# virtualsecureplatform/cuFHE

Hardware: AMD Instinct MI355X
Metric: nand_gate_bootstraps_per_sec (higher is better)
Workload: dtype f64

## Files before the change

### cufhe_amd/csrc/fpfield.h

```cpp
#pragma once
#include <stdint.h>

#if (defined(CUFHE_AMD_ABL_NO_TW) || defined(CUFHE_AMD_ABL_NO_XPOSE) || defined(CUFHE_AMD_ABL_NO_BK) || \
     defined(CUFHE_AMD_ABL_BK0) || defined(CUFHE_AMD_ABL_NO_SYNC) || defined(CUFHE_AMD_ABL_PHASES) || defined(CUFHE_AMD_ABL_LL2_TIMEOUT) || defined(CUFHE_AMD_ABL_L2_NOATOM)) && !defined(CUFHE_AMD_DIAGNOSTIC_BUILD)
#error "CUFHE_AMD_ABL_* switches produce wrong results: use `python cufhe_amd/build.py --diagnostic=NAME[,NAME]` (defines CUFHE_AMD_DIAGNOSTIC_BUILD, output libcufhe_amd_diag.so)"
#endif

#if defined(__HIPCC__)
#define FPF_HD __host__ __device__ __forceinline__
#else
#define FPF_HD static inline
#endif

namespace fpf {

constexpr uint64_t ZETA8 = 5440ull;
constexpr uint64_t P_U64 = 875781160960001ull;
constexpr uint64_t PSI_2048 = 423584205157050ull;
constexpr double P = 875781160960001.0;
constexpr double PINV = 0x1.491cc17c934a8p-50;
constexpr double ROOT4 = 29593600.0;
constexpr double ROOT8 = 5440.0;
constexpr double INV_ROOT4 = 0x1.22436485a6c7fp-25;
constexpr double MAGIC0 = 6755399441055744.0;
constexpr double MAGIC1 = 13510798882111488.0;

FPF_HD double mulmod(double a, double w)
{
    const double h = a * w;
    const double l = __builtin_fma(a, w, -h);
    const double q = __builtin_fma(h, PINV, MAGIC0) - MAGIC0;
    const double r = __builtin_fma(-q, P, h);
    return r + l;
}
FPF_HD double mulmod_wide(double a, double w)
{
    const double h = a * w;
    const double l = __builtin_fma(a, w, -h);
    const double q = __builtin_fma(h, PINV, MAGIC1) - MAGIC1;
    const double r = __builtin_fma(-q, P, h);
    return r + l;
}
FPF_HD double mulmod_add(double a, double w, double c)
{
    const double h = a * w;
    const double l = __builtin_fma(a, w, -h);
    const double q = __builtin_fma(h + c, PINV, MAGIC0) - MAGIC0;
    const double r = __builtin_fma(-q, P, h);
    return (r + c) + l;
}
FPF_HD double mulmod_add_wide(double a, double w, double c)
{
    const double h = a * w;
    const double l = __builtin_fma(a, w, -h);
    const double q = __builtin_fma(h + c, PINV, MAGIC1) - MAGIC1;
    const double r = __builtin_fma(-q, P, h);
    return (r + c) + l;
}
FPF_HD double mul_root4(double x)
{
    const double x1 = __builtin_fma(x, INV_ROOT4, MAGIC0) - MAGIC0;
    const double x0 = __builtin_fma(-x1, ROOT4, x);
    return __builtin_fma(x0, ROOT4, -x1);
}
FPF_HD double reduce(double a)
{
    const double q = __builtin_fma(a, PINV, MAGIC0) - MAGIC0;
    return __builtin_fma(-q, P, a);
}
FPF_HD uint32_t low32(double a)
{
    const double t = a + MAGIC0;
    uint64_t bits;
    __builtin_memcpy(&bits, &t, 8);
    return (uint32_t)bits;
}
FPF_HD uint32_t lift_u32(double a) { return low32(reduce(a)); }
FPF_HD uint32_t lift_u32_small(double a)
{
    const double t = __builtin_fma(a, PINV, MAGIC0);
    uint64_t tb;
    __builtin_memcpy(&tb, &t, 8);
    return low32(a) - (uint32_t)tb * (uint32_t)P_U64;
}


constexpr double GROW = 0.09723;
constexpr double LIM_NARROW = 5.142;
constexpr double LIM_WIDE = 10.285;
constexpr double after_mulmod(double a) { return 0.5 + GROW * a; }
constexpr double after_mulmod_wide(double a) { return 1.0 + GROW * a; }
constexpr double GROW_ADD = 0.14585;
constexpr double after_mulmod_add(double a) { return 0.5 + GROW_ADD * a; }
constexpr double after_mulmod_add_wide(double a) { return 1.0 + GROW_ADD * a; }
constexpr double AFTER_MUL_ROOT4 = 0.5000005;

}
```

### cufhe_amd/csrc/kernels.hip.h

```cpp
#pragma once
#include "kernels_common.hip.h"

namespace cufhe_amd {

__global__ __launch_bounds__(kNttThreads) void bk_to_ntt_kernel(
    double* __restrict__ bk_ntt, const uint32_t* __restrict__ bk, size_t polys,
    const NttTables* __restrict__ gt, double n_inverse)
{
    extern __shared__ __attribute__((aligned(16))) char smem[];
    double* tabs = (double*)smem;
    load_tables_to_lds(tabs, gt);
    __syncthreads();
    const int wave = threadIdx.x >> 6, lane = threadIdx.x & 63;
    const size_t poly = (size_t)blockIdx.x * kNttWavesPerBlock + wave;
    if (poly >= polys) return;
    const WaveCtx ctx = make_wave_ctx(smem, kLdsTableBytes + wave * kTileBytes, 0, gt, lane);
    double x[kRegs];
#pragma unroll
    for (int r = 0; r < kRegs; r++) x[r] = (double)(int32_t)bk[poly * kN + lane + 64 * r];
    ntt_forward<false>(x, ctx);
    double2* dst = (double2*)(bk_ntt + poly * kN);
#pragma unroll
    for (int q = 0; q < 8; q++) {
        double2 v;
        v.x = fpf::reduce(fpf::mulmod_wide(x[2 * q], n_inverse));
        v.y = fpf::reduce(fpf::mulmod_wide(x[2 * q + 1], n_inverse));
        dst[q * 64 + lane] = v;
    }
}

__global__ __launch_bounds__(512) void clock_probe_kernel(double* __restrict__ hz_out, double* __restrict__ sink, int iters)
{
    double x = 1.0 + threadIdx.x * 1e-9, y = 0.5;
    const unsigned long long c0 = __builtin_amdgcn_s_memtime(), r0 = __builtin_amdgcn_s_memrealtime();
#pragma unroll 1
    for (int i = 0; i < iters; i++) {
#pragma unroll
        for (int k = 0; k < 16; k++) { x = __builtin_fma(x, 0.999999, y); y = __builtin_fma(y, 0.999999, x); }
    }
    const unsigned long long c1 = __builtin_amdgcn_s_memtime(), r1 = __builtin_amdgcn_s_memrealtime();
    if (x + y == 12345.678) sink[0] = x;
    if ((threadIdx.x & 63) == 0)
        hz_out[blockIdx.x * (blockDim.x >> 6) + (threadIdx.x >> 6)] = (double)(c1 - c0) / (double)(r1 - r0) * 1.0e8;
}

__device__ __forceinline__ void rotate_sub(uint32_t (&temp)[kRegs], const uint32_t (&acc)[kRegs],
                                           char* tile, int lane, uint32_t abar)
{
    const int alo = (int)(abar & (kN - 1));
    const bool ahi = (abar >> kNbit) != 0;
    char* wpos = tile + opaque(4 * lane + (ahi ? 0 : 4 * kN));
    char* wneg = tile + opaque(4 * lane + (ahi ? 4 * kN : 0));
    asm volatile("" ::: "memory");
#pragma unroll
    for (int r = 0; r < kRegs; r++) {
        *(uint32_t*)(wpos + 256 * r) = acc[r];
        *(uint32_t*)(wneg + 256 * r) = 0u - acc[r];
    }
    asm volatile("" ::: "memory");
    const char* rbase = tile + opaque(4 * (lane - alo + kN));
    uint32_t rot[kRegs];
#pragma unroll
    for (int r = 0; r < kRegs; r++) rot[r] = *(const uint32_t*)(rbase + 256 * r);
#pragma unroll
    for (int r = 0; r < kRegs; r++) temp[r] = (rot[r] - acc[r] + decomp_offset()) ^ decomp_signmask();
}

template <class SPEC, int R, bool LAST, bool FIRST = false>
__device__ __forceinline__ void product_into(double& acc, double x, double w)
{
    constexpr bool wide = r4::needs_wide(SPEC::in().v[R]);
    static_assert(!(LAST && FIRST), "a sum of one product has no first row apart from its last");
    if constexpr (LAST) acc = wide ? fpf::mulmod_add_wide(x, w, acc) : fpf::mulmod_add(x, w, acc);
    else if constexpr (FIRST) acc = wide ? fpf::mulmod_wide(x, w) : fpf::mulmod(x, w);
    else acc += wide ? fpf::mulmod_wide(x, w) : fpf::mulmod(x, w);
}
template <class SPEC, bool LAST, bool FIRST, int Q>
__device__ __forceinline__ void pointwise_piece(double (&A0)[kRegs], double (&A1)[kRegs], const double (&x)[kRegs], const double2& b)
{
    if constexpr (Q < 8) {
        product_into<SPEC, 2 * Q, LAST, FIRST>(A0[2 * Q], x[2 * Q], b.x);
        product_into<SPEC, 2 * Q + 1, LAST, FIRST>(A0[2 * Q + 1], x[2 * Q + 1], b.y);
    } else {
        product_into<SPEC, 2 * (Q - 8), LAST, FIRST>(A1[2 * (Q - 8)], x[2 * (Q - 8)], b.x);
        product_into<SPEC, 2 * (Q - 8) + 1, LAST, FIRST>(A1[2 * (Q - 8) + 1], x[2 * (Q - 8) + 1], b.y);
    }
}
template <class SPEC, bool LAST, bool FIRST, int Q = 0>
__device__ __forceinline__ void pointwise_pieces(double (&A0)[kRegs], double (&A1)[kRegs], const double (&x)[kRegs],
                                                 double2 (&b)[16], const char* row_lane)
{
#ifndef CUFHE_AMD_BK_DEPTH
#define CUFHE_AMD_BK_DEPTH 3
#endif
    constexpr int D = CUFHE_AMD_BK_DEPTH;
    if constexpr (Q < 16) {
        if constexpr (Q + D < 16) b[Q + D] = *(const double2*)(row_lane + (Q + D) * 1024);
        __builtin_amdgcn_sched_barrier(0x0006);
        pointwise_piece<SPEC, LAST, FIRST, Q>(A0, A1, x, b[Q]);
        __builtin_amdgcn_sched_barrier(0x0006);
        pointwise_pieces<SPEC, LAST, FIRST, Q + 1>(A0, A1, x, b, row_lane);
    }
}
template <class SPEC, bool LAST, bool FIRST = false>
__device__ __forceinline__ void pointwise_accumulate(double (&A0)[kRegs], double (&A1)[kRegs],
                                                     const double (&x)[kRegs], const char* row_lane)
{
#if defined(CUFHE_AMD_DIAGNOSTIC_BUILD) && defined(CUFHE_AMD_ABL_NO_BK)
    if constexpr (FIRST) {
#pragma unroll
        for (int r = 0; r < kRegs; r++) { A0[r] = 0.0; A1[r] = 0.0; }
    }
#pragma unroll
    for (int q = 0; q < 8; q++) {
        A0[2 * q] += fpf::mulmod_wide(x[2 * q], 1234567.0 + q);
        A0[2 * q + 1] += fpf::mulmod_wide(x[2 * q + 1], 7654321.0 + q);
        A1[2 * q] += fpf::mulmod_wide(x[2 * q], 2234567.0 + q);
        A1[2 * q + 1] += fpf::mulmod_wide(x[2 * q + 1], 8654321.0 + q);
    }
    (void)row_lane;
    return;
#endif
    constexpr int D = CUFHE_AMD_BK_DEPTH;
    double2 b[16];
#pragma unroll
    for (int q = 0; q < D; q++) b[q] = *(const double2*)(row_lane + q * 1024);
    pointwise_pieces<SPEC, LAST, FIRST>(A0, A1, x, b, row_lane);
}

#if defined(CUFHE_AMD_DIAGNOSTIC_BUILD) && defined(CUFHE_AMD_ABL_PHASES)
#define CUFHE_AMD_DIAG_ARG , unsigned long long& diag_wait
#define CUFHE_AMD_DIAG_PASS , diag_wait
#define CUFHE_AMD_ROW_SYNC(R) { const unsigned long long t0_ = __builtin_readcyclecounter(); pipe.sync(R); diag_wait += __builtin_readcyclecounter() - t0_; }
#else
#define CUFHE_AMD_DIAG_ARG
#define CUFHE_AMD_DIAG_PASS
#define CUFHE_AMD_ROW_SYNC(R) pipe.sync(R);
#endif
struct RowPipe {
    const char* src;
    char* buf;
    uint32_t voff;
    int wave, lane, total_rows;
    bool late;
    int row_off;
    __device__ __forceinline__ RowPipe(const char* bk, char* buf_, int wave_, int lane_, int total_rows_, bool late_)
        : src(bk + 2 * wave_ * 1024), buf(buf_), voff(lane_ * 16), wave(wave_), lane(lane_), total_rows(total_rows_), late(late_),
          row_off((kBkRowBuffers - 1) * kBkRowBytes) {}
    static __device__ __forceinline__ int next_off(int off) { return off == (kBkRowBuffers - 1) * kBkRowBytes ? 0 : off + kBkRowBytes; }
    __device__ __forceinline__ void issue(int R)
    {
        if (R < total_rows) {
            char* dst = buf + next_off(row_off) + 2 * wave * 1024;
#pragma unroll
            for (int c = 0; c < 2; c++) lds_dma16(src + c * 1024, voff, dst + c * 1024);
        }
        src += kBkRowBytes;
    }
    __device__ __forceinline__ void sync(int R)
    {
#if defined(CUFHE_AMD_DIAGNOSTIC_BUILD) && defined(CUFHE_AMD_ABL_NO_SYNC)
        (void)R;
        return;
#endif
        lds_dma_wait_all();
        __syncthreads();
        row_off = next_off(row_off);
        issue(R + 1);
    }
    __device__ __forceinline__ const char* row() const { return buf + opaque(row_off + lane * 16); }
};

using BrSpectrum = r4::FwdDigits<(1 << (kBgbit - 1))>::Spectrum;
using BrSums = r4::PointwiseSum<BrSpectrum, kBkRows, true>;
using BrInverse = r4::Inverse<BrSums>;
static_assert(r4::valid(BrSpectrum::in()) && r4::valid(BrSums::in()) && r4::valid(BrInverse::Out::in()),
              "blind_rotate_kernel: the lazy-reduction schedule of the CMux step exceeds the FP64 mantissa");

template <bool FIRST, bool LAST>
__device__ __forceinline__ void cmux_row(double (&A0)[kRegs], double (&A1)[kRegs], const uint32_t (&temp)[kRegs], int d,
                                         const WaveCtx& ctx, RowPipe& pipe, int row, const TuFwdPinned& tuf CUFHE_AMD_DIAG_ARG)
{
    constexpr int kDigitMax = 1 << (kBgbit - 1);
    const uint32_t pos = 32 - (d + 1) * kBgbit;
    double x[kRegs];
#pragma unroll
    for (int r = 0; r < kRegs; r++)
        x[r] = (double)(int32_t)__builtin_amdgcn_sbfe(temp[r], pos, (uint32_t)kBgbit);
    double twb[kTbCount];
    ntt_forward_digits_a_r4<kDigitMax, true>(x, ctx, &tuf, &twb);
    if (pipe.late) CUFHE_AMD_ROW_SYNC(row)
    ntt_forward_digits_bc_r4<kDigitMax, false, true>(x, ctx, twb);
    if (!pipe.late) CUFHE_AMD_ROW_SYNC(row)
    pointwise_accumulate<BrSpectrum, LAST, FIRST>(A0, A1, x, pipe.row());
}

template <bool FIRST_COMPONENT, bool LAST_COMPONENT>
__device__ __forceinline__ void cmux_component(double (&A0)[kRegs], double (&A1)[kRegs],
                                               const uint32_t (&accj)[kRegs], const WaveCtx& ctx,
                                               char* tile, int lane, uint32_t abar,
                                               RowPipe& pipe, int first_row, const TuFwdPinned& tuf CUFHE_AMD_DIAG_ARG)
{
    uint32_t temp[kRegs];
    rotate_sub(temp, accj, tile, lane, abar);
    static_assert(kL >= 2, "the first and the last row of a component are two rows");
    constexpr int lo = FIRST_COMPONENT ? 1 : 0, hi = LAST_COMPONENT ? kL - 1 : kL;
    if constexpr (FIRST_COMPONENT) cmux_row<true, false>(A0, A1, temp, 0, ctx, pipe, first_row, tuf CUFHE_AMD_DIAG_PASS);
#pragma unroll 1
    for (int d = lo; d < hi; d++) cmux_row<false, false>(A0, A1, temp, d, ctx, pipe, first_row + d, tuf CUFHE_AMD_DIAG_PASS);
    if constexpr (LAST_COMPONENT) cmux_row<false, true>(A0, A1, temp, kL - 1, ctx, pipe, first_row + kL - 1, tuf CUFHE_AMD_DIAG_PASS);
}

template <bool TWB_LOADED>
__device__ __forceinline__ void inverse_and_add(double (&A)[kRegs], uint32_t (&accj)[kRegs], const WaveCtx& ctx,
                                                const double (&twc)[kTcCount], double (&twb)[kTbCount])
{
    ntt_inverse_r4_tw<BrSums, false, TWB_LOADED>(A, ctx, twc, twb);
    lift_add<BrInverse::Out>(accj, A);
}

template <bool TABLE>
__global__ __launch_bounds__(kBrThreads, 2) void blind_rotate_kernel(
    const LinDesc* __restrict__ descs, int count, const double* __restrict__ bk_ntt,
    const NttTables* __restrict__ gt, int steps, uint32_t* __restrict__ acc_dump, int active, const uint32_t* __restrict__ tvs,
    const uint32_t* const* __restrict__ tables)
{
    extern __shared__ __attribute__((aligned(16))) char smem[];
    double* tabs = (double*)(smem + kBrLdsTables);
    load_packed_tables_to_lds(tabs, gt);
    const int wave = __builtin_amdgcn_readfirstlane(threadIdx.x >> 6);
    const int lane = threadIdx.x & 63;
    const int g = blockIdx.x * active + wave;
    char* tile = smem + kBrLdsTiles + wave * kTileBytes;
    uint16_t* abar_lds = (uint16_t*)(smem + kBrLdsAbar + wave * kAbarBytes);
    const WaveCtx ctx = make_wave_ctx_packed(smem, kBrLdsTiles + wave * kTileBytes, kBrLdsTables, gt, lane);
    RowPipe pipe((const char*)bk_ntt, smem + kBrLdsBk, wave, lane, steps * kBkRows, wave >= kBrWavesPerBlock / 2);
    pipe.issue(0);
    if (wave >= active || g >= count) {
        __syncthreads();
#pragma unroll 1
        for (int R = 0; R < pipe.total_rows; R++) pipe.sync(R);
        return;
    }

    const LinDesc d = descs[g];
    uint32_t bword = 0;
#pragma unroll
    for (int rr = 0; rr < 10; rr++) {
        const int i = lane + 64 * rr;
        uint32_t c = 0;
        if (i <= kLvl0N) c = (uint32_t)d.ca * d.in0[i] + (uint32_t)d.cb * d.in1[i];
        if (rr == 9) bword = c;
        if (i < kLvl0N) abar_lds[i] = (uint16_t)((c + (1u << (32 - 2 - kNbit))) >> (32 - 1 - kNbit));
    }
    bword = __builtin_amdgcn_readlane(bword, kLvl0N - 64 * 9) + d.off;
    const uint32_t bbar = 2 * kN - (bword >> (32 - 1 - kNbit));

    uint32_t acc0[kRegs], acc1[kRegs];
#pragma unroll
    for (int r = 0; r < kRegs; r++) {
        const uint32_t e = lane + 64 * r;
        acc0[r] = 0;
        const bool neg = (bbar != 2 * kN) && ((e < (bbar & (kN - 1))) != ((bbar >> kNbit) != 0));
        acc1[r] = neg ? 0u - kMu : kMu;
    }
    const uint32_t* tab = nullptr;
    if constexpr (TABLE) tab = tables[g];
    if (TABLE && tab) {
        const int s = desc_shift(d.pad);
        uint32_t bb = bbar;
        if (s) {
            for (int i = lane; i < kLvl0N; i += 64) abar_lds[i] = (uint16_t)ms_abar((uint32_t)d.ca * d.in0[i] + (uint32_t)d.cb * d.in1[i], s);
            bb = ms_bbar(bword, s);
        }
#pragma unroll
        for (int r = 0; r < kRegs; r++) {
            acc0[r] = rotated_tv_coef(tab, bb, lane + 64 * r);
            acc1[r] = rotated_tv_coef(tab + kN, bb, lane + 64 * r);
        }
    } else if (d.pad) {
        const uint32_t* tv = desc_tv(tvs, d.pad);
        const int s = desc_shift(d.pad);
        uint32_t bb = bbar;
        if (s) {
            for (int i = lane; i < kLvl0N; i += 64) abar_lds[i] = (uint16_t)ms_abar((uint32_t)d.ca * d.in0[i] + (uint32_t)d.cb * d.in1[i], s);
            bb = ms_bbar(bword, s);
        }
#pragma unroll
        for (int r = 0; r < kRegs; r++) acc1[r] = rotated_tv_coef(tv, bb, lane + 64 * r);
    }
    __syncthreads();
    TuFwdPinned tuf;
    tuf.load(gt);
#if defined(CUFHE_AMD_DIAGNOSTIC_BUILD) && defined(CUFHE_AMD_ABL_PHASES)
    unsigned long long diag_wait = 0;
    const unsigned long long diag_t0 = __builtin_readcyclecounter();
#endif

#pragma unroll 1
    for (int i = 0; i < steps; i++) {
        const uint32_t abar = __builtin_amdgcn_readfirstlane((uint32_t)abar_lds[i]);
        double A0[kRegs], A1[kRegs], inv_twc[kTcCount], inv_twb[kTbCount];
        cmux_component<true, false>(A0, A1, acc0, ctx, tile, lane, abar, pipe, i * kBkRows, tuf CUFHE_AMD_DIAG_PASS);
        cmux_component<false, true>(A0, A1, acc1, ctx, tile, lane, abar, pipe, i * kBkRows + kL, tuf CUFHE_AMD_DIAG_PASS);
        load_packed(inv_twc, ctx.tc_inv);
        inverse_and_add<false>(A0, acc0, ctx, inv_twc, inv_twb);
        inverse_and_add<true>(A1, acc1, ctx, inv_twc, inv_twb);
    }

    if (acc_dump) {
        uint32_t* o = acc_dump + (size_t)g * 2 * kN;
#pragma unroll
        for (int r = 0; r < kRegs; r++) {
            o[lane + 64 * r] = acc0[r];
            o[kN + lane + 64 * r] = acc1[r];
        }
#if defined(CUFHE_AMD_DIAGNOSTIC_BUILD) && defined(CUFHE_AMD_ABL_PHASES)
        if (lane == 0) {
            ((unsigned long long*)o)[0] = __builtin_readcyclecounter() - diag_t0;
            ((unsigned long long*)o)[1] = diag_wait;
        }
#endif
    }
    if (d.out) {
        uint32_t* o = d.out;
#pragma unroll
        for (int r = 0; r < kRegs; r++) {
            const int e = lane + 64 * r;
            if (e == 0) { o[0] = acc0[r]; o[kN] = acc1[r]; }
            else o[kN - e] = 0u - acc0[r];
        }
        if (const int s = desc_shift(d.pad)) {
#pragma unroll
            for (int r = 0; r < kRegs; r++) extract_more(o, 1 << s, lane + 64 * r, acc0[r], acc1[r]);
        }
    }
}

constexpr int kKsWaves = 16;
constexpr int kKsThreads = 64 * kKsWaves;
constexpr int kKsRowPad = 640;
constexpr int kKsPieces = 3;
constexpr int kKsStepBytes = kKsT * kKsNumBase * kKsRowPad * 4;
constexpr int kKsBuffers = 3;
constexpr int kKsDigitSteps = 1024;
constexpr int kKsLdsDigits = kKsWaves * kKsDigitSteps * 2;

struct KsShapeDefault {
    using Desc = LinDesc;
    static constexpr int kn = kN, t = kKsT, row_pad = kKsRowPad, n_out = kLvl0N;
    static constexpr uint32_t koff()
    {
        uint32_t o = 1u << (32 - (1 + kKsBasebit * kKsT));
        for (int i = 1; i <= kKsT; i++) o += ((1u << kKsBasebit) / 2) << (32 - i * kKsBasebit);
        return o;
    }
    static __device__ __forceinline__ uint32_t digit_word(const Desc& d, int j)
    {
        return ((uint32_t)d.ca * d.in0[j] + (uint32_t)d.cb * d.in1[j] + koff()) >> 16;
    }
    static __device__ __forceinline__ uint32_t bprime(const Desc& d) { return (uint32_t)d.ca * d.in0[kn] + (uint32_t)d.cb * d.in1[kn] + d.off; }
};
template <class S>
struct KsDims {
    static constexpr int pairs = (S::row_pad - 512) / 128;
    static constexpr int words = 8 + 2 * pairs;
    static constexpr int step_bytes = S::t * kKsNumBase * S::row_pad * 4;
    static constexpr int dma_pieces = step_bytes / 1024;
    static constexpr int dma_more = dma_pieces - 2 * kKsWaves;
    static constexpr int lds_bytes = kKsLdsDigits + kKsBuffers * step_bytes;
    static constexpr int min_slices = (S::kn + kKsDigitSteps - 1) / kKsDigitSteps;
// ... 503 lines not shown
```

### cufhe_amd/csrc/ntt_r4.h

```cpp
#pragma once
#include "fpfield.h"

#if defined(__HIPCC__)
#define R4_HD __host__ __device__ __forceinline__
#else
#define R4_HD inline
#endif

namespace cufhe_amd {
namespace r4 {

struct RegBounds {
    double v[16];
};
constexpr double kPoison = 1.0e30;
constexpr double kReduced = 0.5001;

constexpr RegBounds uniform(double b)
{
    RegBounds r{};
    for (int i = 0; i < 16; i++) r.v[i] = b;
    return r;
}
constexpr double max_of(const RegBounds& b)
{
    double m = 0;
    for (int i = 0; i < 16; i++) m = b.v[i] > m ? b.v[i] : m;
    return m;
}
constexpr bool valid(const RegBounds& b) { return max_of(b) < fpf::LIM_WIDE; }
constexpr bool needs_wide(double b) { return b >= fpf::LIM_NARROW; }
constexpr double after_product(double b)
{
    return b >= fpf::LIM_WIDE ? kPoison : needs_wide(b) ? fpf::after_mulmod_wide(b) : fpf::after_mulmod(b);
}
constexpr double checked(double b) { return b >= fpf::LIM_WIDE ? kPoison : b; }

template <bool HI>
constexpr int reg_of(int group, int coarse, int fine)
{
    return HI ? group + 8 * coarse + 4 * fine : 4 * group + 2 * coarse + fine;
}

template <bool HI>
constexpr RegBounds ct_bounds(const RegBounds& in)
{
    RegBounds out{};
    for (int g = 0; g < 4; g++) {
        const double a = in.v[reg_of<HI>(g, 0, 0)];
        const double mb = after_product(in.v[reg_of<HI>(g, 1, 0)]);
        const double mc = after_product(in.v[reg_of<HI>(g, 0, 1)]);
        const double md = after_product(in.v[reg_of<HI>(g, 1, 1)]);
        const double sum = checked(checked(a + mb) + checked(mc + md));
        const double dif = checked(checked(a + mb) + fpf::AFTER_MUL_ROOT4);
        out.v[reg_of<HI>(g, 0, 0)] = sum;
        out.v[reg_of<HI>(g, 0, 1)] = sum;
        out.v[reg_of<HI>(g, 1, 0)] = dif;
        out.v[reg_of<HI>(g, 1, 1)] = dif;
    }
    return out;
}
template <bool HI>
constexpr RegBounds gs_bounds(const RegBounds& in)
{
    RegBounds out{};
    for (int g = 0; g < 4; g++) {
        const double s0 = checked(in.v[reg_of<HI>(g, 0, 0)] + in.v[reg_of<HI>(g, 0, 1)]);
        const double s1 = checked(in.v[reg_of<HI>(g, 1, 0)] + in.v[reg_of<HI>(g, 1, 1)]);
        out.v[reg_of<HI>(g, 0, 0)] = checked(s0 + s1);
        out.v[reg_of<HI>(g, 1, 0)] = after_product(checked(s0 + s1));
        out.v[reg_of<HI>(g, 0, 1)] = after_product(checked(s0 + fpf::AFTER_MUL_ROOT4));
        out.v[reg_of<HI>(g, 1, 1)] = after_product(checked(s0 + fpf::AFTER_MUL_ROOT4));
    }
    return out;
}
constexpr RegBounds xpose_all_bounds(const RegBounds& in) { return uniform(max_of(in)); }
constexpr RegBounds xpose_bc_bounds(const RegBounds& in)
{
    RegBounds out{};
    for (int m = 0; m < 4; m++) {
        double mx = 0;
        for (int h = 0; h < 4; h++) mx = in.v[4 * h + m] > mx ? in.v[4 * h + m] : mx;
        for (int g = 0; g < 4; g++) out.v[4 * m + g] = mx;
    }
    return out;
}
constexpr RegBounds xpose_cb_bounds(const RegBounds& in)
{
    RegBounds out{};
    for (int m = 0; m < 4; m++) {
        double mx = 0;
        for (int g = 0; g < 4; g++) mx = in.v[4 * m + g] > mx ? in.v[4 * m + g] : mx;
        for (int h = 0; h < 4; h++) out.v[4 * h + m] = mx;
    }
    return out;
}
constexpr RegBounds reduce_bounds(const RegBounds& in, double limit)
{
    RegBounds out = in;
    for (int r = 0; r < 16; r++)
        if (in.v[r] > limit) out.v[r] = kReduced;
    return out;
}
constexpr RegBounds reduce_mask_bounds(const RegBounds& in, unsigned mask)
{
    RegBounds out = in;
    for (int r = 0; r < 16; r++)
        if ((mask >> r) & 1u) out.v[r] = kReduced;
    return out;
}

template <class S, bool HI>
struct AfterCt {
    static constexpr RegBounds in() { return ct_bounds<HI>(S::in()); }
};
template <class S, bool HI>
struct AfterGs {
    static constexpr RegBounds in() { return gs_bounds<HI>(S::in()); }
};
template <class S>
struct AfterXposeAll {
    static constexpr RegBounds in() { return xpose_all_bounds(S::in()); }
};
template <class S>
struct AfterXposeBC {
    static constexpr RegBounds in() { return xpose_bc_bounds(S::in()); }
};
template <class S>
struct AfterXposeCB {
    static constexpr RegBounds in() { return xpose_cb_bounds(S::in()); }
};
template <class S, int LIMIT_MILLI>
struct AfterReduce {
    static constexpr RegBounds in() { return reduce_bounds(S::in(), LIMIT_MILLI * 0.001); }
};
template <class S, unsigned MASK>
struct AfterReduceMask {
    static constexpr RegBounds in() { return reduce_mask_bounds(S::in(), MASK); }
};
template <int MILLI>
struct Uniform {
    static constexpr RegBounds in() { return uniform(MILLI * 0.001); }
};

template <int DIGIT_MAX>
struct DigitsAfterExact {
    static constexpr RegBounds in()
    {
        const double s1 = DIGIT_MAX * (1.0 + fpf::ROOT4 + fpf::ROOT8 + fpf::ROOT8 * fpf::ROOT8 * fpf::ROOT8);
        return uniform(s1 < 9007199254740992.0 / 64.0 ? s1 / fpf::P : kPoison);
    }
};
template <int DIGIT_MAX>
struct FwdDigits {
    using A0 = DigitsAfterExact<DIGIT_MAX>;
    using B0 = AfterXposeAll<AfterCt<A0, false>>;
    using B1 = AfterCt<B0, true>;
    using C0 = AfterXposeBC<AfterCt<B1, false>>;
    static constexpr unsigned kReduceC = 0x1111u;
    using C1 = AfterReduceMask<C0, kReduceC>;
    using Spectrum = AfterCt<C1, false>;
};
template <class SPEC, int ROWS, bool FUSED>
struct PointwiseSum {
    static constexpr RegBounds in()
    {
        RegBounds out{};
        const RegBounds s = SPEC::in();
        for (int r = 0; r < 16; r++) {
            const double prod = after_product(s.v[r]);
            if (FUSED) {
                const double last = s.v[r] >= fpf::LIM_WIDE ? kPoison : needs_wide(s.v[r]) ? fpf::after_mulmod_add_wide(s.v[r]) : fpf::after_mulmod_add(s.v[r]);
                out.v[r] = checked((ROWS - 1) * prod + last) >= kPoison ? kPoison : last;
            } else {
                out.v[r] = checked(ROWS * prod);
            }
        }
        return out;
    }
};

template <class S0>
struct Inverse {
    static constexpr int kLimit = 2570;
    using C1 = AfterGs<S0, false>;
    using B0 = AfterXposeCB<AfterReduce<C1, kLimit>>;
    using B1 = AfterReduce<AfterGs<B0, false>, kLimit>;
    using B2 = AfterReduce<AfterGs<B1, true>, kLimit>;
    using A0 = AfterXposeAll<B2>;
    using A1 = AfterReduce<AfterGs<A0, false>, kLimit>;
    using Out = AfterGs<A1, true>;
};

template <bool WIDE>
R4_HD double product(double a, double w) { return WIDE ? fpf::mulmod_wide(a, w) : fpf::mulmod(a, w); }

template <bool WB, bool WC, bool WD>
R4_HD void ct_bfly4(double& x0, double& xf, double& xc, double& xcf, double w, double u, double uw)
{
    const double b = product<WB>(xc, w), c = product<WC>(xf, u), d = product<WD>(xcf, uw);
    const double s = x0 + b, e = x0 - b, t = c + d, v = fpf::mul_root4(c - d);
    x0 = s + t;
    xf = s - t;
    xc = e + v;
    xcf = e - v;
}
template <bool WC, bool WF, bool WCF>
R4_HD void gs_bfly4(double& x0, double& xf, double& xc, double& xcf, double w, double v, double vw)
{
    const double s0 = x0 + xf, p = x0 - xf, s1 = xc + xcf, q = fpf::mul_root4(xc - xcf);
    x0 = s0 + s1;
    xc = product<WC>(s0 - s1, w);
    xf = product<WF>(p - q, v);
    xcf = product<WCF>(p + q, vw);
}

template <class S, bool HI, int G>
struct Group {
    static constexpr RegBounds b = S::in();
    static constexpr int r0 = reg_of<HI>(G, 0, 0), rf = reg_of<HI>(G, 0, 1), rc = reg_of<HI>(G, 1, 0), rcf = reg_of<HI>(G, 1, 1);
    static R4_HD void ct(double (&x)[16], double w, double u, double uw)
    {
        ct_bfly4<needs_wide(b.v[rc]), needs_wide(b.v[rf]), needs_wide(b.v[rcf])>(x[r0], x[rf], x[rc], x[rcf], w, u, uw);
    }
    static R4_HD void gs(double (&x)[16], double w, double v, double vw)
    {
        constexpr double s0 = b.v[r0] + b.v[rf], s1 = b.v[rc] + b.v[rcf];
        gs_bfly4<needs_wide(s0 + s1), needs_wide(s0 + fpf::AFTER_MUL_ROOT4), needs_wide(s0 + fpf::AFTER_MUL_ROOT4)>(x[r0], x[rf], x[rc], x[rcf], w, v, vw);
    }
};

template <class S, class TW>
R4_HD void ct_pass_hi(double (&x)[16], const TW& tw)
{
    const double w = tw(0), u = tw(1), uw = tw(2);
    Group<S, true, 0>::ct(x, w, u, uw);
    Group<S, true, 1>::ct(x, w, u, uw);
    Group<S, true, 2>::ct(x, w, u, uw);
    Group<S, true, 3>::ct(x, w, u, uw);
}
template <class S, int WB, int UB, class TW>
R4_HD void ct_pass_lo(double (&x)[16], const TW& tw)
{
    Group<S, false, 0>::ct(x, tw(WB + 0), tw(UB + 0), tw(UB + 1));
    Group<S, false, 1>::ct(x, tw(WB + 1), tw(UB + 2), tw(UB + 3));
    Group<S, false, 2>::ct(x, tw(WB + 2), tw(UB + 4), tw(UB + 5));
    Group<S, false, 3>::ct(x, tw(WB + 3), tw(UB + 6), tw(UB + 7));
}
template <class S, class TW>
R4_HD void gs_pass_hi(double (&x)[16], const TW& tw)
{
    const double w = tw(0), v = tw(1), vw = tw(2);
    Group<S, true, 0>::gs(x, w, v, vw);
    Group<S, true, 1>::gs(x, w, v, vw);
    Group<S, true, 2>::gs(x, w, v, vw);
    Group<S, true, 3>::gs(x, w, v, vw);
}
template <class S, int WB, int UB, class TW>
R4_HD void gs_pass_lo(double (&x)[16], const TW& tw)
{
    Group<S, false, 0>::gs(x, tw(WB + 0), tw(UB + 0), tw(UB + 1));
    Group<S, false, 1>::gs(x, tw(WB + 1), tw(UB + 2), tw(UB + 3));
    Group<S, false, 2>::gs(x, tw(WB + 2), tw(UB + 4), tw(UB + 5));
    Group<S, false, 3>::gs(x, tw(WB + 3), tw(UB + 6), tw(UB + 7));
}
template <class S, int LIMIT_MILLI, int R = 0>
R4_HD void reduce_above(double (&x)[16])
{
    if constexpr (R < 16) {
        if constexpr (S::in().v[R] > LIMIT_MILLI * 0.001) x[R] = fpf::reduce(x[R]);
        reduce_above<S, LIMIT_MILLI, R + 1>(x);
    }
}

template <class S, int LIMIT_MILLI, int G>
R4_HD void reduce_above_group(double (&x)[16])
{
    if constexpr (S::in().v[G] > LIMIT_MILLI * 0.001) x[G] = fpf::reduce(x[G]);
    if constexpr (S::in().v[G + 4] > LIMIT_MILLI * 0.001) x[G + 4] = fpf::reduce(x[G + 4]);
    if constexpr (S::in().v[G + 8] > LIMIT_MILLI * 0.001) x[G + 8] = fpf::reduce(x[G + 8]);
    if constexpr (S::in().v[G + 12] > LIMIT_MILLI * 0.001) x[G + 12] = fpf::reduce(x[G + 12]);
}
template <unsigned MASK, int R = 0>
R4_HD void reduce_mask(double (&x)[16])
{
    if constexpr (R < 16) {
        if constexpr (((MASK >> R) & 1u) != 0) x[R] = fpf::reduce(x[R]);
        reduce_mask<MASK, R + 1>(x);
    }
}

}
}
```

### cufhe_amd/csrc/ntt_wave.h

```cpp
#pragma once
#include <hip/hip_runtime.h>
#include "fpfield.h"
#include "ntt_r4.h"
#include "ntt_tables.h"

namespace cufhe_amd {

constexpr int kRegs = 16;
constexpr int kTileSlots = 66 * 16;
constexpr int kTileBytes = kTileSlots * 8;

constexpr double forward_digit_spectrum_bound(double digit_max)
{
    const double s1 = digit_max * (1.0 + fpf::ROOT4 + fpf::ROOT8 + fpf::ROOT8 * fpf::ROOT8 * fpf::ROOT8);
    if (s1 >= 9007199254740992.0 / 64.0) return -1.0;
    double b = s1 / fpf::P;
    for (int s = 2; s <= 8; s++) {
        if (b >= fpf::LIM_NARROW) return -1.0;
        b = b + fpf::after_mulmod(b);
    }
    if (b >= fpf::LIM_WIDE) return -1.0;
    return b + fpf::after_mulmod_wide(b);
}
constexpr double forward_words_spectrum_bound()
{
    double b = 4294967296.0 / fpf::P;
    for (int s = 0; s <= 7; s++) {
        if (b >= fpf::LIM_NARROW) return -1.0;
        b = b + fpf::after_mulmod(b);
    }
    for (int s = 8; s <= 9; s++) {
        if (b >= fpf::LIM_WIDE) return -1.0;
        b = b + fpf::after_mulmod_wide(b);
    }
    return b;
}
static_assert(forward_words_spectrum_bound() > 0 && forward_words_spectrum_bound() < fpf::LIM_WIDE, "forward NTT schedule (32-bit words in)");
constexpr bool pointwise_sum_fits(double s, int rows)
{
    return s > 0 && s < fpf::LIM_WIDE && rows * fpf::after_mulmod_wide(s) < fpf::LIM_WIDE;
}
constexpr double inverse_output_bound()
{
    double b = 0.5001;
    for (int s = 0; s < 2; s++) {
        if (2 * b >= fpf::LIM_NARROW) return -1.0;
        b = 2 * b;
    }
    for (int half = 0; half < 2; half++) {
        if (2 * b >= fpf::LIM_NARROW) return -1.0;
        b = 2 * b;
        if (2 * b >= fpf::LIM_WIDE) return -1.0;
        b = 2 * b;
        b = 0.5001;
        for (int s = 0; s < 2; s++) {
            if (2 * b >= fpf::LIM_NARROW) return -1.0;
            b = 2 * b;
        }
    }
    return b;
}
constexpr bool inverse_schedule_fits() { return inverse_output_bound() > 0 && inverse_output_bound() < 2.57; }
static_assert(inverse_schedule_fits(), "inverse NTT lazy-reduction schedule exceeds the FP64 mantissa");


__device__ __forceinline__ void load_tables_to_lds(double* lds, const NttTables* g)
{
    const double* src = g->tb_fwd;
    for (int i = threadIdx.x; i < kLdsTableDoubles; i += blockDim.x) lds[i] = src[i];
}

__device__ __forceinline__ void load_packed_tables_to_lds(double* lds, const NttTables* g)
{
    const double* src = g->tbp_fwd;
    for (int i = threadIdx.x; i < kLdsTablePackedDoubles; i += blockDim.x) lds[i] = src[i];
}

struct WaveCtx {
    char* a65;
    char* a66;
    char* b65;
    char* b66;
    const char* tb_fwd;
    const char* tb_inv;
    const char* tc_fwd;
    const char* tc_inv;
    const NttTables* gt;
    const char* tu_l;
};

__device__ __forceinline__ void lds_dma16(const void* src, char* dst_uniform)
{
    const uint32_t base = (uint32_t)(uintptr_t)(__attribute__((address_space(3))) void*)dst_uniform;
#pragma clang diagnostic push
#pragma clang diagnostic ignored "-Winline-asm"
    asm volatile("s_mov_b32 m0, %1\n\ts_nop 0\n\tglobal_load_lds_dwordx4 %0, off" ::"v"(src), "s"(base) : "memory", "m0");
#pragma clang diagnostic pop
}
__device__ __forceinline__ void lds_dma16(const char* src_uniform, uint32_t voff, char* dst_uniform)
{
    const uint32_t base = (uint32_t)(uintptr_t)(__attribute__((address_space(3))) void*)dst_uniform;
#pragma clang diagnostic push
#pragma clang diagnostic ignored "-Winline-asm"
    asm volatile("s_mov_b32 m0, %2\n\ts_nop 0\n\tglobal_load_lds_dwordx4 %0, %1" ::"v"(voff), "s"(src_uniform), "s"(base) : "memory", "m0");
#pragma clang diagnostic pop
}
__device__ __forceinline__ void lds_dma_wait_all() { asm volatile("s_waitcnt vmcnt(0)" ::: "memory"); }

__device__ __forceinline__ int opaque(int off)
{
    asm volatile("" : "+v"(off));
    return off;
}

__device__ __forceinline__ WaveCtx make_wave_ctx(char* lds, int tile_off, int tables_off,
                                                 const NttTables* gt, int lane)
{
    const int lam = lane & 15, hi = lane >> 4;
    WaveCtx c;
    c.a65 = lds + opaque(tile_off + 8 * lane);
    c.a66 = c.a65;
    c.b65 = lds + opaque(tile_off + 8 * (65 * lam + hi));
    c.b66 = lds + opaque(tile_off + 8 * (66 * lam + hi));
    c.tb_fwd = lds + opaque(tables_off + 8 * lam);
    c.tb_inv = c.tb_fwd + 8 * (kTbCount * 16);
    c.tc_fwd = lds + opaque(tables_off + 8 * (2 * kTbCount * 16) + 8 * lane);
    c.tc_inv = c.tc_fwd + 8 * (kTcCount * 64);
    c.gt = gt;
    c.tu_l = nullptr;
    return c;
}

__device__ __forceinline__ WaveCtx make_wave_ctx_packed(char* lds, int tile_off, int tables_off, const NttTables* gt, int lane)
{
    WaveCtx c = make_wave_ctx(lds, tile_off, tables_off, gt, lane);
    c.tb_fwd = lds + opaque(tables_off + 8 * kTbpStride * (lane & 15));
    c.tb_inv = c.tb_fwd + 8 * 16 * kTbpStride;
    c.tc_fwd = lds + opaque(tables_off + 8 * 2 * 16 * kTbpStride + 8 * kTcpStride * lane);
    c.tc_inv = c.tc_fwd + 8 * 64 * kTcpStride;
    return c;
}
__device__ __forceinline__ double2 lds_ld2(const char* p, int off) { return *(const double2*)(p + off); }
template <int COUNT>
__device__ __forceinline__ void load_packed(double (&tw)[COUNT], const char* base)
{
#pragma unroll
    for (int i = 0; i < (COUNT + 1) / 2; i++) {
        const double2 v = lds_ld2(base, 16 * i);
        tw[2 * i] = v.x;
        if (2 * i + 1 < COUNT) tw[2 * i + 1] = v.y;
    }
}
#if defined(CUFHE_AMD_DIAGNOSTIC_BUILD) && defined(CUFHE_AMD_ABL_NO_TW)
__device__ __forceinline__ double lds_ld(const char* p, int off) { return 12345678.0 + (double)off + (double)(uintptr_t)p * 1e-30; }
// ... 266 lines not shown
template <bool WIDE8, bool HALF_TILE = false>
__device__ __forceinline__ void ntt_forward_bc(double (&x)[kRegs], const WaveCtx& c)
{
    double twb[kTbCount];
#pragma unroll
    for (int k = 0; k < kTbCount; k++) twb[k] = lds_ld(c.tb_fwd, 128 * k);
    if (HALF_TILE) xpose_half_tile<true>(x, c.a66, c.b66);
    else CUFHE_AMD_XPOSE(c.a66, 8 * 66, c.b66, 32)
    ct_four_stages<false>(x, TwArr{twb});
    double twc[kTcCount];
#pragma unroll
    for (int k = 0; k < kTcCount; k++) twc[k] = lds_ld(c.tc_fwd, 512 * k);
    xpose_bc_permlane(x);
#pragma unroll
    for (int g = 0; g < 4; g++) {
#pragma unroll
        for (int r = 0; r < 2; r++) ct_bfly<WIDE8>(x[4 * g + r], x[4 * g + r + 2], twc[g]);
    }
#pragma unroll
    for (int g = 0; g < 8; g++) ct_bfly<true>(x[2 * g], x[2 * g + 1], twc[4 + g]);
}
template <bool SMALL_IN, bool HALF_TILE = false>
__device__ __forceinline__ void ntt_forward(double (&x)[kRegs], const WaveCtx& c)
{
    ntt_forward_a<SMALL_IN>(x, c);
    ntt_forward_bc<!SMALL_IN, HALF_TILE>(x, c);
}

template <bool HALF_TILE = false, bool TU_LDS = false>
__device__ __forceinline__ void ntt_inverse_twc(double (&x)[kRegs], const WaveCtx& c, const double (&twc)[kTcCount])
{
#pragma unroll
    for (int g = 0; g < 8; g++) gs_bfly<false>(x[2 * g], x[2 * g + 1], twc[4 + g]);
#pragma unroll
    for (int g = 0; g < 4; g++) {
#pragma unroll
        for (int r = 0; r < 2; r++) gs_bfly<false>(x[4 * g + r], x[4 * g + r + 2], twc[g]);
    }
    double twb[kTbCount];
#pragma unroll
    for (int k = 0; k < kTbCount; k++) twb[k] = lds_ld(c.tb_inv, 128 * k);
    xpose_cb_permlane(x);
    gs_four_stages(x, TwArr{twb});
    double tu[15];
    if (TU_LDS) load_tu(tu, c.tu_l + 128);
    if (HALF_TILE) xpose_half_tile<false>(x, c.a65, c.b65);
    else CUFHE_AMD_XPOSE(c.b65, 32, c.a65, 8 * 65)
    if (TU_LDS) gs_four_stages(x, TwArr{tu});
    else gs_four_stages(x, TwUniform{c.gt->tu_inv});
}
template <bool HALF_TILE = false, bool TU_LDS = false>
__device__ __forceinline__ void ntt_inverse2_twc(double (&x)[kRegs], double (&y)[kRegs], const WaveCtx& c, const double (&twc)[kTcCount])
{
    gs_stage<1, false>(x, TwArr{twc}, 4);
    gs_stage<1, false>(y, TwArr{twc}, 4);
    gs_stage<2, false>(x, TwArr{twc}, 0);
    gs_stage<2, false>(y, TwArr{twc}, 0);
    double twb[kTbCount];
#pragma unroll
    for (int k = 0; k < kTbCount; k++) twb[k] = lds_ld(c.tb_inv, 128 * k);
    xpose_cb_permlane(x);
    xpose_cb_permlane(y);
    gs_four_stages2(x, y, TwArr{twb});
    double tu[15];
    if (TU_LDS) load_tu(tu, c.tu_l + 128);
    if (HALF_TILE) { xpose_half_tile<false>(x, c.a65, c.b65); xpose_half_tile<false>(y, c.a65, c.b65); }
    else { CUFHE_AMD_XPOSE(c.b65, 32, c.a65, 8 * 65) { double (&x)[kRegs] = y; CUFHE_AMD_XPOSE(c.b65, 32, c.a65, 8 * 65) } }
    if (TU_LDS) gs_four_stages2(x, y, TwArr{tu});
    else gs_four_stages2(x, y, TwUniform{c.gt->tu_inv});
}
template <bool HALF_TILE = false, bool TU_LDS = false>
__device__ __forceinline__ void ntt_inverse(double (&x)[kRegs], const WaveCtx& c)
{
    double twc[kTcCount];
#pragma unroll
    for (int k = 0; k < kTcCount; k++) twc[k] = lds_ld(c.tc_inv, 512 * k);
    ntt_inverse_twc<HALF_TILE, TU_LDS>(x, c, twc);
}



struct TuFwdPinned {
    double t[12];
    double root4, root8;
    __device__ __forceinline__ void load(const NttTables* gt)
    {
#pragma unroll
        for (int k = 0; k < 12; k++) {
            double v = gt->tu_fwd[3 + k];
            asm volatile("" : "+s"(v));
            t[k] = v;
        }
        root4 = fpf::ROOT4;
        root8 = fpf::ROOT8;
        asm volatile("" : "+s"(root4), "+s"(root8));
    }
    __device__ __forceinline__ double operator()(int k) const { return t[k - 3]; }
};
template <int DIGIT_MAX, bool STORE = false, class TW = TwUniform>
__device__ __forceinline__ void ntt_forward_digits_a_r4(double (&x)[kRegs], const WaveCtx& c, const TW* pinned = nullptr, double (*twb_ahead)[kTbCount] = nullptr)
{
    using A0 = typename r4::FwdDigits<DIGIT_MAX>::A0;
    if constexpr (!STORE) {
        ct_exact_first_two(x);
        r4::ct_pass_lo<A0, 3, 7>(x, TwUniform{c.gt->tu_fwd});
    } else {
        const TW& tw = *pinned;
        ct_exact_first_two(x, tw.root4, tw.root8);
        if (twb_ahead) load_packed(*twb_ahead, c.tb_fwd);
        asm volatile("" ::: "memory");
        r4::Group<A0, false, 0>::ct(x, tw(3), tw(7), tw(8));
#pragma unroll
        for (int r = 0; r < 4; r++) lds_st(c.a66, 8 * 66 * r, x[r]);
        r4::Group<A0, false, 1>::ct(x, tw(4), tw(9), tw(10));
#pragma unroll
        for (int r = 4; r < 8; r++) lds_st(c.a66, 8 * 66 * r, x[r]);
        r4::Group<A0, false, 2>::ct(x, tw(5), tw(11), tw(12));
#pragma unroll
        for (int r = 8; r < 12; r++) lds_st(c.a66, 8 * 66 * r, x[r]);
        r4::Group<A0, false, 3>::ct(x, tw(6), tw(13), tw(14));
#pragma unroll
        for (int r = 12; r < 16; r++) lds_st(c.a66, 8 * 66 * r, x[r]);
    }
}
template <int DIGIT_MAX, bool HALF_TILE = false, bool STORED = false>
__device__ __forceinline__ void ntt_forward_digits_bc_r4(double (&x)[kRegs], const WaveCtx& c, const double* twb_loaded = nullptr)
{
    using F = r4::FwdDigits<DIGIT_MAX>;
    static_assert(r4::valid(F::Spectrum::in()), "radix-4 forward transform of gadget digits: a value exceeds 2^53");
    static_assert(!(HALF_TILE && STORED), "the half-size tile takes the layout change in two passes");
    double twb[kTbCount];
    if (twb_loaded) {
#pragma unroll
        for (int k = 0; k < kTbCount; k++) twb[k] = twb_loaded[k];
    } else {
        load_packed(twb, c.tb_fwd);
    }
    if (HALF_TILE) xpose_half_tile<true>(x, c.a66, c.b66);
    else if (STORED) {
        asm volatile("" ::: "memory");
#pragma unroll
        for (int r = 0; r < kRegs; r++) x[r] = lds_ld(c.b66, 32 * r);
    }
    else CUFHE_AMD_XPOSE(c.a66, 8 * 66, c.b66, 32)
    r4::ct_pass_hi<typename F::B0>(x, TwArr{twb});
    r4::ct_pass_lo<typename F::B1, 3, 7>(x, TwArr{twb});
    double twc[kTcCount];
    load_packed(twc, c.tc_fwd);
    xpose_bc_permlane(x);
    r4::reduce_mask<F::kReduceC>(x);
    r4::ct_pass_lo<typename F::C1, 0, 4>(x, TwArr{twc});
}

template <class S0, bool HALF_TILE, bool TWB_LOADED>
__device__ __forceinline__ void ntt_inverse_r4_tw(double (&x)[kRegs], const WaveCtx& c, const double (&twc)[kTcCount], double (&twb)[kTbCount]);
template <class S0, bool HALF_TILE = false>
__device__ __forceinline__ void ntt_inverse_r4(double (&x)[kRegs], const WaveCtx& c)
{
    double twc[kTcCount], twb[kTbCount];
    load_packed(twc, c.tc_inv);
    ntt_inverse_r4_tw<S0, HALF_TILE, false>(x, c, twc, twb);
}
template <class S0, bool HALF_TILE, bool TWB_LOADED>
__device__ __forceinline__ void ntt_inverse_r4_tw(double (&x)[kRegs], const WaveCtx& c, const double (&twc)[kTcCount], double (&twb)[kTbCount])
{
    using V = r4::Inverse<S0>;
    static_assert(r4::valid(V::Out::in()), "radix-4 inverse transform: a value exceeds 2^53");
    r4::gs_pass_lo<S0, 0, 4>(x, TwArr{twc});
    r4::reduce_above<typename V::C1, V::kLimit>(x);
    if (!TWB_LOADED) load_packed(twb, c.tb_inv);
    xpose_cb_permlane(x);
    r4::gs_pass_lo<typename V::B0, 3, 7>(x, TwArr{twb});
    r4::reduce_above<r4::AfterGs<typename V::B0, false>, V::kLimit>(x);
    if (HALF_TILE) {
        r4::gs_pass_hi<typename V::B1>(x, TwArr{twb});
        r4::reduce_above<r4::AfterGs<typename V::B1, true>, V::kLimit>(x);
        xpose_half_tile<false>(x, c.a65, c.b65);
    } else {
        using B1o = r4::AfterGs<typename V::B1, true>;
        const double w = twb[0], v = twb[1], vw = twb[2];
        double tu[15];
#pragma unroll
        for (int k = 0; k < 15; k++) tu[k] = c.gt->tu_inv[k];
        asm volatile("" ::: "memory");
        r4::Group<typename V::B1, true, 0>::gs(x, w, v, vw);
        r4::reduce_above_group<B1o, V::kLimit, 0>(x);
#pragma unroll
        for (int k = 0; k < 16; k += 4) lds_st(c.b65, 32 * k, x[k]);
        r4::Group<typename V::B1, true, 1>::gs(x, w, v, vw);
        r4::reduce_above_group<B1o, V::kLimit, 1>(x);
#pragma unroll
        for (int k = 1; k < 16; k += 4) lds_st(c.b65, 32 * k, x[k]);
        r4::Group<typename V::B1, true, 2>::gs(x, w, v, vw);
        r4::reduce_above_group<B1o, V::kLimit, 2>(x);
#pragma unroll
        for (int k = 2; k < 16; k += 4) lds_st(c.b65, 32 * k, x[k]);
        r4::Group<typename V::B1, true, 3>::gs(x, w, v, vw);
        r4::reduce_above_group<B1o, V::kLimit, 3>(x);
#pragma unroll
        for (int k = 3; k < 16; k += 4) lds_st(c.b65, 32 * k, x[k]);
        asm volatile("" ::: "memory");
#pragma unroll
        for (int r = 0; r < kRegs; r++) x[r] = lds_ld(c.a65, 8 * 65 * r);
        r4::gs_pass_lo<typename V::A0, 3, 7>(x, TwArr{tu});
        r4::reduce_above<r4::AfterGs<typename V::A0, false>, V::kLimit>(x);
        r4::gs_pass_hi<typename V::A1>(x, TwArr{tu});
        return;
    }
    r4::gs_pass_lo<typename V::A0, 3, 7>(x, TwUniform{c.gt->tu_inv});
    r4::reduce_above<r4::AfterGs<typename V::A0, false>, V::kLimit>(x);
    r4::gs_pass_hi<typename V::A1>(x, TwUniform{c.gt->tu_inv});
}
template <class OUT, int R = 0>
__device__ __forceinline__ void lift_add(uint32_t (&acc)[kRegs], const double (&x)[kRegs])
{
    if constexpr (R < kRegs) {
        if constexpr (OUT::in().v[R] < 2.57) acc[R] += fpf::lift_u32_small(x[R]);
        else acc[R] += fpf::lift_u32(x[R]);
        lift_add<OUT, R + 1>(acc, x);
    }
}

}
```

Measured before the change: 114,800.

## Specialize last inverse NTT pass with constant-root products and cheaper lift

Adds a dedicated tail for the blind-rotate inverse NTT. The final radix-4 GS pass multiplies by fixed 8th/4th roots using split-constant tricks instead of generic twiddle mulmods, so the uniform tu_inv twiddles for that pass no longer need loading. Reductions now follow explicit per-register masks instead of reduce_above. The lift-add skips the final modular reduction wherever static bounds show the value is already within range. This lowers FP64 op count and register pressure in the hot CMux loop, but relies on tighter constexpr bound reasoning about the sums.

Measured after the change: 116,500 (median of 6 runs). 1.02x the previous value.

```diff
diff --git a/cufhe_amd/csrc/fpfield.h b/cufhe_amd/csrc/fpfield.h
--- a/cufhe_amd/csrc/fpfield.h
+++ b/cufhe_amd/csrc/fpfield.h
@@ -22,6 +22,9 @@
 constexpr double ROOT4 = 29593600.0;
 constexpr double ROOT8 = 5440.0;
 constexpr double INV_ROOT4 = 0x1.22436485a6c7fp-25;
+constexpr double ROOT8_CUBED = 160989184000.0;
+constexpr double INV_ROOT8 = 0x1.8181818181818p-13;
+constexpr double INV_ROOT8_CUBED = 0x1.b51a30f9739f8p-38;
 constexpr double MAGIC0 = 6755399441055744.0;
 constexpr double MAGIC1 = 13510798882111488.0;
 
@@ -63,6 +66,18 @@
     const double x0 = __builtin_fma(-x1, ROOT4, x);
     return __builtin_fma(x0, ROOT4, -x1);
 }
+FPF_HD double mul_root8(double x)
+{
+    const double x1 = __builtin_fma(x, INV_ROOT8_CUBED, MAGIC0) - MAGIC0;
+    const double x0 = __builtin_fma(-x1, ROOT8_CUBED, x);
+    return __builtin_fma(x0, ROOT8, -x1);
+}
+FPF_HD double mul_root8_cubed(double x)
+{
+    const double x1 = __builtin_fma(x, INV_ROOT8, MAGIC0) - MAGIC0;
+    const double x0 = __builtin_fma(-x1, ROOT8, x);
+    return __builtin_fma(x0, ROOT8_CUBED, -x1);
+}
 FPF_HD double reduce(double a)
 {
     const double q = __builtin_fma(a, PINV, MAGIC0) - MAGIC0;
@@ -83,7 +98,7 @@
     __builtin_memcpy(&tb, &t, 8);
     return low32(a) - (uint32_t)tb * (uint32_t)P_U64;
 }
-
+FPF_HD uint32_t lift_u32_reduced(double a) { return low32(a); }
 
 constexpr double GROW = 0.09723;
 constexpr double LIM_NARROW = 5.142;
@@ -94,5 +109,8 @@
 constexpr double after_mulmod_add(double a) { return 0.5 + GROW_ADD * a; }
 constexpr double after_mulmod_add_wide(double a) { return 1.0 + GROW_ADD * a; }
 constexpr double AFTER_MUL_ROOT4 = 0.5000005;
+constexpr double AFTER_MUL_ROOT8 = 0.5000001;
+constexpr double AFTER_MUL_ROOT8_CUBED = 0.5021;
+constexpr bool lift_reduced_ok(double b, double cmax) { return b + cmax < 1.0; }
 
 }
diff --git a/cufhe_amd/csrc/kernels.hip.h b/cufhe_amd/csrc/kernels.hip.h
--- a/cufhe_amd/csrc/kernels.hip.h
+++ b/cufhe_amd/csrc/kernels.hip.h
@@ -173,9 +173,11 @@
 
 using BrSpectrum = r4::FwdDigits<(1 << (kBgbit - 1))>::Spectrum;
 using BrSums = r4::PointwiseSum<BrSpectrum, kBkRows, true>;
-using BrInverse = r4::Inverse<BrSums>;
+using BrInverse = r4::InverseRootTail6x32<BrSums>;
 static_assert(r4::valid(BrSpectrum::in()) && r4::valid(BrSums::in()) && r4::valid(BrInverse::Out::in()),
               "blind_rotate_kernel: the lazy-reduction schedule of the CMux step exceeds the FP64 mantissa");
+constexpr int kBrTrueMaxMilli = (int)(kExtProdSumBound / fpf::P * 1000.0) + 1;
+static_assert(kBrTrueMaxMilli < 500, "the sums of the CMux step must stay below p/2");
 
 template <bool FIRST, bool LAST>
 __device__ __forceinline__ void cmux_row(double (&A0)[kRegs], double (&A1)[kRegs], const uint32_t (&temp)[kRegs], int d,
@@ -215,8 +217,8 @@
 __device__ __forceinline__ void inverse_and_add(double (&A)[kRegs], uint32_t (&accj)[kRegs], const WaveCtx& ctx,
                                                 const double (&twc)[kTcCount], double (&twb)[kTbCount])
 {
-    ntt_inverse_r4_tw<BrSums, false, TWB_LOADED>(A, ctx, twc, twb);
-    lift_add<BrInverse::Out>(accj, A);
+    ntt_inverse_r4_tw<BrSums, false, TWB_LOADED, BrInverse>(A, ctx, twc, twb);
+    lift_add_fp64<BrInverse::Out, kBrTrueMaxMilli>(accj, A);
 }
 
 template <bool TABLE>
diff --git a/cufhe_amd/csrc/ntt_r4.h b/cufhe_amd/csrc/ntt_r4.h
--- a/cufhe_amd/csrc/ntt_r4.h
+++ b/cufhe_amd/csrc/ntt_r4.h
@@ -74,6 +74,20 @@
     }
     return out;
 }
+constexpr RegBounds gs_last_bounds(const RegBounds& in)
+{
+    RegBounds out{};
+    for (int g = 0; g < 4; g++) {
+        const double s0 = checked(in.v[reg_of<true>(g, 0, 0)] + in.v[reg_of<true>(g, 0, 1)]);
+        const double s1 = checked(in.v[reg_of<true>(g, 1, 0)] + in.v[reg_of<true>(g, 1, 1)]);
+        const bool fits = checked(s0 + s1) < kPoison && checked(s0 + fpf::AFTER_MUL_ROOT4) < kPoison;
+        out.v[reg_of<true>(g, 0, 0)] = checked(s0 + s1);
+        out.v[reg_of<true>(g, 1, 0)] = fits ? fpf::AFTER_MUL_ROOT4 : kPoison;
+        out.v[reg_of<true>(g, 0, 1)] = fits ? fpf::AFTER_MUL_ROOT8_CUBED : kPoison;
+        out.v[reg_of<true>(g, 1, 1)] = fits ? fpf::AFTER_MUL_ROOT8 : kPoison;
+    }
+    return out;
+}
 constexpr RegBounds xpose_all_bounds(const RegBounds& in) { return uniform(max_of(in)); }
 constexpr RegBounds xpose_bc_bounds(const RegBounds& in)
 {
@@ -117,6 +131,10 @@
 template <class S, bool HI>
 struct AfterGs {
     static constexpr RegBounds in() { return gs_bounds<HI>(S::in()); }
+};
+template <class S>
+struct AfterGsLast {
+    static constexpr RegBounds in() { return gs_last_bounds(S::in()); }
 };
 template <class S>
 struct AfterXposeAll {
@@ -192,6 +210,21 @@
     using Out = AfterGs<A1, true>;
 };
 
+template <class S0, unsigned MC1, unsigned MB0, unsigned MB1, unsigned MA0>
+struct InverseRootTail {
+    static constexpr unsigned kMaskC1 = MC1, kMaskB0 = MB0, kMaskB1 = MB1, kMaskA0 = MA0;
+    using In = S0;
+    using C1 = AfterGs<S0, false>;
+    using B0 = AfterXposeCB<AfterReduceMask<C1, MC1>>;
+    using B1 = AfterReduceMask<AfterGs<B0, false>, MB0>;
+    using B2 = AfterReduceMask<AfterGs<B1, true>, MB1>;
+    using A0 = AfterXposeAll<B2>;
+    using A1 = AfterReduceMask<AfterGs<A0, false>, MA0>;
+    using Out = AfterGsLast<A1>;
+};
+template <class S0>
+using InverseRootTail6x32 = InverseRootTail<S0, 0x0011u, 0x1111u, 0x000eu, 0x0111u>;
+
 template <bool WIDE>
 R4_HD double product(double a, double w) { return WIDE ? fpf::mulmod_wide(a, w) : fpf::mulmod(a, w); }
 
@@ -213,6 +246,14 @@
     xc = product<WC>(s0 - s1, w);
     xf = product<WF>(p - q, v);
     xcf = product<WCF>(p + q, vw);
+}
+R4_HD void gs_bfly4_last(double& x0, double& xf, double& xc, double& xcf)
+{
+    const double s0 = x0 + xf, np = xf - x0, s1 = xc + xcf, q = fpf::mul_root4(xc - xcf);
+    x0 = s0 + s1;
+    xc = fpf::mul_root4(s1 - s0);
+    xf = fpf::mul_root8_cubed(np + q);
+    xcf = fpf::mul_root8(np - q);
 }
 
 template <class S, bool HI, int G>
@@ -256,6 +297,15 @@
     Group<S, true, 2>::gs(x, w, v, vw);
     Group<S, true, 3>::gs(x, w, v, vw);
 }
+template <class S>
+R4_HD void gs_pass_hi_last(double (&x)[16])
+{
+    static_assert(valid(gs_last_bounds(S::in())), "last inverse pass: a sum exceeds 2^53");
+    gs_bfly4_last(x[0], x[4], x[8], x[12]);
+    gs_bfly4_last(x[1], x[5], x[9], x[13]);
+    gs_bfly4_last(x[2], x[6], x[10], x[14]);
+    gs_bfly4_last(x[3], x[7], x[11], x[15]);
+}
 template <class S, int WB, int UB, class TW>
 R4_HD void gs_pass_lo(double (&x)[16], const TW& tw)
 {
diff --git a/cufhe_amd/csrc/ntt_wave.h b/cufhe_amd/csrc/ntt_wave.h
--- a/cufhe_amd/csrc/ntt_wave.h
+++ b/cufhe_amd/csrc/ntt_wave.h
@@ -1,5 +1,6 @@
 #pragma once
 #include <hip/hip_runtime.h>
+#include <type_traits>
 #include "fpfield.h"
 #include "ntt_r4.h"
 #include "ntt_tables.h"
@@ -572,7 +573,7 @@
     r4::ct_pass_lo<typename F::C1, 0, 4>(x, TwArr{twc});
 }
 
-template <class S0, bool HALF_TILE, bool TWB_LOADED>
+template <class S0, bool HALF_TILE, bool TWB_LOADED, class TAIL = void>
 __device__ __forceinline__ void ntt_inverse_r4_tw(double (&x)[kRegs], const WaveCtx& c, const double (&twc)[kTcCount], double (&twb)[kTbCount]);
 template <class S0, bool HALF_TILE = false>
 __device__ __forceinline__ void ntt_inverse_r4(double (&x)[kRegs], const WaveCtx& c)
@@ -581,9 +582,52 @@
     load_packed(twc, c.tc_inv);
     ntt_inverse_r4_tw<S0, HALF_TILE, false>(x, c, twc, twb);
 }
-template <class S0, bool HALF_TILE, bool TWB_LOADED>
+template <class V, bool TWB_LOADED>
+__device__ __forceinline__ void ntt_inverse_r4_root_tail(double (&x)[kRegs], const WaveCtx& c, const double (&twc)[kTcCount], double (&twb)[kTbCount])
+{
+    static_assert(r4::valid(V::Out::in()), "radix-4 inverse transform (root products in the last pass): a value exceeds 2^53");
+    r4::gs_pass_lo<typename V::In, 0, 4>(x, TwArr{twc});
+    r4::reduce_mask<V::kMaskC1>(x);
+    if (!TWB_LOADED) load_packed(twb, c.tb_inv);
+    xpose_cb_permlane(x);
+    r4::gs_pass_lo<typename V::B0, 3, 7>(x, TwArr{twb});
+    r4::reduce_mask<V::kMaskB0>(x);
+    const double w = twb[0], v = twb[1], vw = twb[2];
+    double tu[15];
+#pragma unroll
+    for (int k = 3; k < 15; k++) tu[k] = c.gt->tu_inv[k];
+    asm volatile("" ::: "memory");
+    r4::Group<typename V::B1, true, 0>::gs(x, w, v, vw);
+    r4::reduce_mask<V::kMaskB1 & 0x1111u>(x);
+#pragma unroll
+    for (int k = 0; k < 16; k += 4) lds_st(c.b65, 32 * k, x[k]);
+    r4::Group<typename V::B1, true, 1>::gs(x, w, v, vw);
+    r4::reduce_mask<V::kMaskB1 & 0x2222u>(x);
+#pragma unroll
+    for (int k = 1; k < 16; k += 4) lds_st(c.b65, 32 * k, x[k]);
+    r4::Group<typename V::B1, true, 2>::gs(x, w, v, vw);
+    r4::reduce_mask<V::kMaskB1 & 0x4444u>(x);
+#pragma unroll
+    for (int k = 2; k < 16; k += 4) lds_st(c.b65, 32 * k, x[k]);
+    r4::Group<typename V::B1, true, 3>::gs(x, w, v, vw);
+    r4::reduce_mask<V::kMaskB1 & 0x8888u>(x);
+#pragma unroll
+    for (int k = 3; k < 16; k += 4) lds_st(c.b65, 32 * k, x[k]);
+    asm volatile("" ::: "memory");
+#pragma unroll
+    for (int r = 0; r < kRegs; r++) x[r] = lds_ld(c.a65, 8 * 65 * r);
+    r4::gs_pass_lo<typename V::A0, 3, 7>(x, TwArr{tu});
+    r4::reduce_mask<V::kMaskA0>(x);
+    r4::gs_pass_hi_last<typename V::A1>(x);
+}
+template <class S0, bool HALF_TILE, bool TWB_LOADED, class TAIL>
 __device__ __forceinline__ void ntt_inverse_r4_tw(double (&x)[kRegs], const WaveCtx& c, const double (&twc)[kTcCount], double (&twb)[kTbCount])
 {
+    if constexpr (!std::is_void<TAIL>::value) {
+        static_assert(!HALF_TILE && std::is_same<typename TAIL::In, S0>::value, "the root-product tail: full tile, and the schedule of this input");
+        ntt_inverse_r4_root_tail<TAIL, TWB_LOADED>(x, c, twc, twb);
+        return;
+    }
     using V = r4::Inverse<S0>;
     static_assert(r4::valid(V::Out::in()), "radix-4 inverse transform: a value exceeds 2^53");
     r4::gs_pass_lo<S0, 0, 4>(x, TwArr{twc});
@@ -631,6 +675,15 @@
     r4::reduce_above<r4::AfterGs<typename V::A0, false>, V::kLimit>(x);
     r4::gs_pass_hi<typename V::A1>(x, TwUniform{c.gt->tu_inv});
 }
+template <class OUT, int TRUE_MAX_MILLI, int R = 0>
+__device__ __forceinline__ void lift_add_fp64(uint32_t (&acc)[kRegs], const double (&x)[kRegs])
+{
+    if constexpr (R < kRegs) {
+        if constexpr (fpf::lift_reduced_ok(OUT::in().v[R], TRUE_MAX_MILLI * 0.001)) acc[R] += fpf::lift_u32_reduced(x[R]);
+        else acc[R] += fpf::lift_u32(x[R]);
+        lift_add_fp64<OUT, TRUE_MAX_MILLI, R + 1>(acc, x);
+    }
+}
 template <class OUT, int R = 0>
 __device__ __forceinline__ void lift_add(uint32_t (&acc)[kRegs], const double (&x)[kRegs])
 {
```
